# SomeBottle/LinearProgramming

Hardware: AMD Instinct MI355X
Metric: Simplex pivots/sec + HBM GB/s fraction, dense m=16384×n=32768 fp64, 1/2/4/8 GPU (higher is better)
Workload: dtype f64

## Files before the change

### linearprogramming_amd/csrc/lpg_ctx.hip

```cpp
#include <hip/hip_runtime.h>
#include <rccl/rccl.h>

#include <dlfcn.h>
#include <unistd.h>
#include <math.h>
#include <stdarg.h>
#include <stdio.h>
#include <stdlib.h>
#include <string.h>

#include <algorithm>
#include <vector>

#include "../../include/lpg.h"
#include "lpg_internal.h"

using namespace lpg;

namespace {

thread_local char g_err[512];

struct TimingRing {
    std::vector<hipEvent_t> ev;
// ... 238 lines not shown
    t.used = 0;
    return 0;
}

static int timing_mark(lpg_ctx *c, int which, int updated = 1) {
    TimingRing &t = c->tr;
    if (which == 0 && t.used * 3 + 3 > (int)t.ev.size()) {
        int rc = timing_flush(c);
        if (rc) return rc;
    }
    HIPCHK(c, hipEventRecord(t.ev[3 * t.used + which], c->stream));
    if (which == 2) t.upd[t.used++] = (char)updated;
    return 0;
}


static Defer defer_of(const lpg_ctx *c, int q) {
    Defer d;
    d.Pbuf = c->Pbuf;
    d.Cbuf = c->Cbuf;
    d.cs = c->cs;
    d.rq = c->rq;
    d.rqg = c->rqg;
    d.basis = c->basis;
    d.logk = c->logk;
    d.logr = c->logr;
    d.zrow = c->zrow;
    d.kq = c->kq;
    d.lv = c->lv;
    d.colmap = c->colmap;
    d.inv = c->inv;
    d.mul = c->mul;
    d.pv = c->pv;
    d.q = q;
    d.on = c->defer_k > 0 ? 1 : 0;
    return d;
}

static bool reorders(const lpg_ctx *c) { return c->defer_k > 0 && c->fast_pivot && c->colmap && !c->no_reorder; }

#ifdef LPG_TEST_HOOKS
static int inject_pending_fault(lpg_ctx *c) {
    switch (c->inject_what) {
        case 1: HIPCHK(c, hipMemsetAsync(&c->st->npend, 0x7f, sizeof(int64_t), c->stream)); break;
        case 2: HIPCHK(c, hipMemsetAsync(c->kq, 0xff, sizeof(int64_t), c->stream)); break;
        case 3: HIPCHK(c, hipMemsetAsync(c->lv, 0xff, sizeof(int64_t), c->stream)); break;
        case 4: HIPCHK(c, hipMemsetAsync(c->rq, 0x7f, sizeof(int64_t), c->stream)); break;
        case 5: {
            HIPCHK(c, hipStreamSynchronize(c->stream));
            int64_t np = 0;
            HIPCHK(c, hipMemcpy(&np, &c->st->npend, sizeof np, hipMemcpyDeviceToHost));
            np += 1;
            HIPCHK(c, hipMemcpy(&c->st->npend, &np, sizeof np, hipMemcpyHostToDevice));
            break;
        }
        default: break;
    }
    return 0;
}

#endif

static int flush_launch(lpg_ctx *c) {
    int rc;
    const bool re = reorders(c);
#ifdef LPG_TEST_HOOKS
    if (c->inject_flush >= 0 && c->nflush == c->inject_flush && (rc = inject_pending_fault(c))) return rc;
#endif
    c->nflush++;
    const int unit = (c->block_region && c->reg_valid && c->move_unit) ? 1 : 0;
    if (launch_swap_plan(lau(c), geo(c), c->st, defer_of(c, 0), c->colmap, c->inv, c->pairs, re ? 1 : 0, c->defer_k) ||
        (re && launch_move_cols(lau(c), geo(c), c->st, defer_of(c, 0), c->pairs, unit)))
        return fail(c, LPG_ERR_DEVICE, "swap plan launch failed");
#ifdef LPG_TEST_HOOKS
    if (c->inject_rbad >= 0 && c->nflush == c->inject_rbad + 1)
        HIPCHK(c, hipMemsetAsync(&c->st->rbad, 0x01, sizeof(uint32_t), c->stream));
#endif
    if (c->timing && ((rc = timing_mark(c, 0)) || (rc = timing_mark(c, 1)))) return rc;
    const int32_t *tl = (c->block_region && c->reg_valid && re && c->tlive_on && c->skip) ? c->tlive : nullptr;
    c->block_region = false;
    if (launch_flush_main(lau(c), geo(c), c->st, defer_of(c, 0), c->pend, c->skip, c->flush_variant, c->flush_xcd, tl))
        return fail(c, LPG_ERR_DEVICE, "flush launch failed");
    if (c->timing && (rc = timing_mark(c, 2, 2))) return rc;
    if (launch_flush_tail(lau(c), geo(c), c->st, defer_of(c, 0), c->pend, !re))
        return fail(c, LPG_ERR_DEVICE, "flush launch failed");
    if (re) {
        const Defer D = defer_of(c, 0);
        if (launch_fill_cols(lau(c), geo(c), c->pairs, c->st, &D, flush_kmax_supported(c->defer_k),
                             c->reg ? c->bcol0 : nullptr))
            return fail(c, LPG_ERR_DEVICE, "fill launch failed");
        c->permuted = true;
    }
    c->pend = 0;
    return 0;
}

static int materialize(lpg_ctx *c) {
    if (c->defer_k == 0 || c->pend == 0) return 0;
    return flush_launch(c);
}

static int canonicalize(lpg_ctx *c) {
    int rc = materialize(c);
    c->reg_valid = false;
    if (rc || !c->permuted) return rc;
    const int64_t rows = c->nloc + c->nobj;
    if (!c->tmp) {
        c->tmp_rows = std::min<int64_t>(rows, 512);
        HIPCHK(c, hipMalloc(&c->tmp, (size_t)c->tmp_rows * c->ld * sizeof(double)));
    }
    const Geo g = geo(c);
    for (int64_t i0 = 0; i0 < rows; i0 += c->tmp_rows) {
        const int64_t nr = std::min(c->tmp_rows, rows - i0);
        if (launch_gather_rows(lau(c), g, c->inv, c->tmp, i0, nr)) return fail(c, LPG_ERR_DEVICE, "gather launch failed");
        HIPCHK(c, hipMemcpy2DAsync(c->T + i0 * c->ld, c->ld * sizeof(double), c->tmp, c->ld * sizeof(double),
                                   c->ncols * sizeof(double), nr, hipMemcpyDeviceToDevice, c->stream));
    }
    if (launch_iota(lau(c), c->colmap, c->ld) || launch_iota(lau(c), c->inv, c->ld))
        return fail(c, LPG_ERR_DEVICE, "iota launch failed");
    c->permuted = false;
    return 0;
}


static int cand_per_rank(const lpg_ctx *c) { return (c->defer_k > 0 && c->fast_pivot) ? c->nsel_d : c->nsel; }

static int64_t prow_count(const lpg_ctx *c) { return (c->ncols + 1) & ~(int64_t)1; }

static int exchange_candidates(lpg_ctx *c) {
    if (!has_comm(c)) return 0;
    return comm_allgather(c, c->part, c->cand, sizeof(Cand) * (size_t)cand_per_rank(c));
}

static int clear_candidates(lpg_ctx *c) {
    if (c->nsel_d > c->nsel)
        HIPCHK(c, hipMemsetAsync(c->part + c->nsel, 0xff, (size_t)(c->nsel_d - c->nsel) * sizeof(Cand), c->stream));
    return 0;
}

static int region_setup(lpg_ctx *c);

static int bootstrap(lpg_ctx *c, int rule) {
    int rc = canonicalize(c);
    if (rc || (rc = region_setup(c)) || (rc = clear_candidates(c))) return rc;
    HIPCHK(c, hipMemsetAsync(c->st->slot, 0, sizeof(c->st->slot), c->stream));
    const Geo g = geo(c);
    if (launch_price(lau(c), g, rule, 0, c->st, 0, c->P, c->C[0], c->pp, c->pc, c->npp))
        return fail(c, LPG_ERR_DEVICE, "price launch failed");
    if (launch_select(lau(c), g, rule, true, c->st, 0, 0, c->P, c->C[1], c->C[0], c->pp, c->npp, c->basis,
                      c->part, c->nsel, 0, -1, c->pc, c->skip, defer_of(c, 0)))
        return fail(c, LPG_ERR_DEVICE, "select launch failed");
    if ((rc = exchange_candidates(c))) return rc;
    c->par = 0;
    c->booted = true;
    c->boot_rule = rule;
    c->x_from_cand = true;
    return 0;
}

static int bootstrap_forced(lpg_ctx *c, int rule, int64_t k, int64_t r) {
    int rc = canonicalize(c);
    if (rc || (rc = region_setup(c)) || (rc = clear_candidates(c))) return rc;
    HIPCHK(c, hipMemsetAsync(c->st->slot, 0, sizeof(c->st->slot), c->stream));
    if (launch_select(lau(c), geo(c), rule, true, c->st, 0, 0, c->P, c->C[1], c->C[0], c->pp, c->npp, c->basis,
                      c->part, c->nsel, k, r, c->pc, c->skip, defer_of(c, 0)))
        return fail(c, LPG_ERR_DEVICE, "select launch failed");
    if ((rc = exchange_candidates(c))) return rc;
    c->par = 0;
    c->booted = true;
    c->boot_rule = rule;
    c->x_from_cand = true;
    return 0;
}

static constexpr int kGraphPivots = 32;
// ... 1427 lines not shown
```

### linearprogramming_amd/csrc/lpg_internal.h

```cpp
#pragma once
#include <stddef.h>
#include <stdint.h>

namespace lpg {

constexpr int kBlock = 256;
constexpr int kMaxSelBlocks = 512;
#ifndef LPG_DEFER_MAX
#define LPG_DEFER_MAX 128
#endif

enum : int32_t { RUNNING = 0, OPTIMAL = 1, UNBOUNDED = 2, INFEASIBLE = 3, ITER_LIMIT = 4, NUMERIC = 5 };
enum : int { RULE_DANTZIG = 0, RULE_BLAND = 1 };

struct Slot {
    int64_t k;
    int64_t r;
    int32_t status;
    int32_t pad0;
    int64_t dpend;
};

struct DevState {
    Slot    slot[2];
// ... 48 lines not shown

struct Cand {
    double  theta;
    double  piv;
    int64_t key;
    int64_t row;
};

struct PricePart {
    double  v;
    int64_t j;
    int32_t cls;
    int32_t pad;
};

struct Geo {
    double *T;
    int64_t ld;
    int64_t nloc;
    int64_t nobj;
    int64_t ncols;
    int64_t nact;
    int64_t row0;
    int64_t m;
    double  eps_piv, eps_opt;
};

struct Launch {
    void   *stream;
};

int launch_generate(const Launch &L, const Geo &g, int64_t n, uint64_t seed, int kind, int64_t *basis_dev);
int launch_objective_chain(const Launch &L, const Geo &g, const double *cb, const double *acc_in, double *acc_out);
int launch_objective_finish(const Launch &L, const Geo &g, const double *acc, const double *cost, int64_t orow);
int launch_price(const Launch &L, const Geo &g, int rule, int mode, const DevState *st, int s,
                 const double *P, const double *Cs, PricePart *pp, int *pc, int npp, bool defer = false,
                 const int32_t *colmap = nullptr, const int32_t *inv = nullptr);
int launch_prep(const Launch &L, const Geo &g, int rule, bool fuse_price, DevState *st, int s,
                const Cand *cand, int ncand, double *P, const double *Cs, PricePart *pp, int *pc, int npp,
                const Defer &D);
int launch_select(const Launch &L, const Geo &g, int rule, bool first, DevState *st, int s, int s1,
                  const double *P, const double *Cs, double *Cs1, const PricePart *pp, int npp,
                  const int64_t *basis, Cand *part, int nsel, int64_t force_k, int64_t force_r,
                  const int *pc, int skip, const Defer &D);
constexpr int kPivotThreads = 256;
int pivot_d_blocks(const Geo &g, int which, int nt);
int launch_pivot_d(const Launch &L, const Geo &g, int rule, DevState *st, int s, int s1, Cand *part, int nsel,
                   double *P, const double *Cs, double *Cs1, PricePart *pp, int npp, const int64_t *basis,
                   const Defer &D, int nt);
int launch_prep_dm(const Launch &L, const Geo &g, int rule, DevState *st, int s, const Cand *cand, int ncand,
                   double *P, const double *Cs, int npp_d, const Defer &D);
int launch_prep_x(const Launch &L, const Geo &g, int rule, DevState *st, int s, const Cand *cand, int ncand,
                  double *P, const double *Cs, PricePart *pp, int npp_d, const Defer &D, const Xch &X);
int launch_select_x(const Launch &L, const Geo &g, int rule, DevState *st, int s, int s1, const double *Cs,
                    double *Cs1, const PricePart *pp, int npp, const int64_t *basis, Cand *part, int nsel,
                    const Defer &D, const Xch &X);
int64_t xch_bytes(int64_t ld, int world, int nblk, int nx, int64_t *offF, int64_t *offC, int64_t *offG);
int launch_select_dm(const Launch &L, const Geo &g, int rule, DevState *st, int s, int s1, const double *Cs,
                     double *Cs1, const PricePart *pp, int npp, const int64_t *basis, Cand *part, int nsel,
                     const Defer &D);
int block_records_bytes(int nwg);
int block_geometry(const Geo &g, int ks, int cus, int want, int *nwg, int *cw, int *rw, size_t *lds);
struct RegionGeo {
    int nwg, cw, rw, nsp, cwx;
    size_t lds;
};
struct RegionArgs {
    const int32_t *live;
    int64_t nlive;
    const int64_t *bcol0;
    int nsp, cwx;
};
int block_geometry_region(const Geo &g, int ks, int cus, int want, int64_t nlive, RegionGeo *out);
int launch_region_build(const Launch &L, const Geo &g, DevState *st, const int64_t *basis, const int32_t *inv,
                        int32_t *mark, int32_t *live, int64_t *bcol0, int64_t nlive, int32_t *tlive);
int launch_region_check(const Launch &L, const Geo &g, const int64_t *basis, const int32_t *inv, int *ok);
int launch_pivot_block(const Launch &L, const Geo &g, int rule, DevState *st, int s0, int q0, int n, Cand *part,
                       int ncand, const Cand *cin, int ncin, const double *Cs0, double *Cs1, const Defer &D,
                       void *rec, uint32_t tag0, int nwg, int cw, int rw, int ks, size_t lds, uint32_t cl,
                       const Xch *X = nullptr, uint32_t xtag0 = 0, const RegionArgs *R = nullptr);
int launch_flush(const Launch &L, const Geo &g, DevState *st, const Defer &D, int kmax, int skip, int which);
int launch_flush_main(const Launch &L, const Geo &g, DevState *st, const Defer &D, int kmax, int skip, int which,
                      int xcd = -1, const int32_t *tlive = nullptr);
int launch_flush_tail(const Launch &L, const Geo &g, DevState *st, const Defer &D, int kmax, bool reset = true);
__host__ __device__ inline int64_t flush_tail_rows(int64_t rows, int64_t nloc) {
    return (rows > 0 && nloc >= 8 * rows && rows >= 64) ? rows / 4 : 0;
}
__host__ __device__ inline int64_t flush_nitems(int64_t ntiles, int64_t rows, int64_t nloc) {
    const int64_t tr = flush_tail_rows(rows, nloc);
    if (rows < 0) rows = -rows;
    if (!tr) return ntiles * ((nloc + rows - 1) / rows);
    const int64_t t0 = ((nloc + rows - 1) / rows - 2) * rows;
    return ntiles * (t0 / rows) + ntiles * ((nloc - t0 + tr - 1) / tr);
}
__host__ __device__ inline void flush_item(int64_t item, int64_t ntiles, int64_t rows, int64_t nloc, int64_t &tile,
                                           int64_t &i0, int64_t &i1) {
    const int64_t tr = flush_tail_rows(rows, nloc);
    if (rows < 0) rows = -rows;
    const int64_t t0 = tr ? ((nloc + rows - 1) / rows - 2) * rows : nloc;
    const int64_t nbig = ntiles * (t0 / rows);
    tile = item % ntiles;
    if (!tr || item < nbig) {
        i0 = (item / ntiles) * rows;
        i1 = i0 + rows;
    } else {
        i0 = t0 + ((item - nbig) / ntiles) * tr;
        i1 = i0 + tr;
    }
    if (i1 > nloc) i1 = nloc;
}
struct FlushX {
    int64_t ntiles, nloc;
    int32_t H;
    int32_t rb;
    int32_t rs;
    int32_t tt;
    int32_t on;
    int32_t tq;
};
struct FlushXGroup {
    int64_t r0, r1, ntg, nsb, ttg, nq, qrows, count;
};
__host__ __device__ inline FlushXGroup flushx_group(const FlushX &f, int g) {
    FlushXGroup o{};
    const int b = g / f.H, h = g % f.H;
    o.r0 = (int64_t)b * f.rb;
    o.r1 = o.r0 + f.rb < f.nloc ? o.r0 + f.rb : f.nloc;
    o.ntg = h < f.ntiles ? (f.ntiles - h + f.H - 1) / f.H : 0;
    if (o.r0 >= f.nloc || o.ntg == 0) return o;
    o.nsb = (o.r1 - o.r0 + f.rs - 1) / f.rs;
    const int64_t ls = (o.r1 - o.r0) - (o.nsb - 1) * f.rs;
    const int64_t tq = f.tq > 0 ? f.tq : 4;
    o.qrows = ((ls + tq - 1) / tq + 15) / 16 * 16;
    o.nq = (ls + o.qrows - 1) / o.qrows;
    o.ttg = f.tt < o.ntg ? f.tt : o.ntg;
    o.count = (o.nsb - 1) * o.ntg + (o.ntg - o.ttg) + o.nq * o.ttg;
    return o;
}
__host__ __device__ inline void flushx_item(const FlushX &f, const FlushXGroup &G, int g, int64_t it, int64_t &tile,
                                            int64_t &i0, int64_t &i1) {
    const int h = g % f.H;
    int64_t j;
    const int64_t full = (G.nsb - 1) * G.ntg;
    const int64_t base = G.r0 + (G.nsb - 1) * f.rs;
    if (it < full) {
        j = G.ntg - 1 - it % G.ntg;
        i0 = G.r0 + (it / G.ntg) * f.rs;
        i1 = i0 + f.rs;
    } else if (it - full < G.ntg - G.ttg) {
        j = G.ntg - 1 - (it - full);
        i0 = base;
        i1 = G.r1;
    } else {
        const int64_t k = it - full - (G.ntg - G.ttg);
        j = G.ttg - 1 - k / G.nq;
        i0 = base + (k % G.nq) * G.qrows;
        i1 = i0 + G.qrows;
    }
    if (i1 > G.r1) i1 = G.r1;
    tile = h + (int64_t)f.H * j;
}
int flush_kmax_supported(int k);
int launch_swap_plan(const Launch &L, const Geo &g, DevState *st, const Defer &D, int32_t *colmap, int32_t *inv,
                     int32_t *pairs, int plan, int kmax);
constexpr int kPairW = 4;
int launch_move_cols(const Launch &L, const Geo &g, const DevState *st, const Defer &D, const int32_t *pairs,
                     int unit);
int launch_fill_cols(const Launch &L, const Geo &g, const int32_t *pairs, DevState *st = nullptr,
                     const Defer *D = nullptr, int kmax = 0, int64_t *bcol0 = nullptr);
int launch_gather_rows(const Launch &L, const Geo &g, const int32_t *inv, double *tmp, int64_t i0, int64_t nr);
int launch_iota(const Launch &L, int32_t *a, int64_t n);
int launch_update(const Launch &L, const Geo &g, DevState *st, int s, const double *P, const double *Cs,
                  int64_t *basis, int64_t *logk, int64_t *logr, int variant, int skip);

int launch_dual_rows(const Launch &L, const Geo &g, Cand *part, int nsel);
int launch_dual_row_d(const Launch &L, const Geo &g, DevState *st, int s, const Cand *rc, int nrc, Cand *cp,
                      double *R, const double *Pprev, const double *Cprev, const Defer &D, bool mr);
int launch_dual_ratio(const Launch &L, const Geo &g, const DevState *st, int s, const double *R, Cand *cp);
int launch_dual_col_d(const Launch &L, const Geo &g, DevState *st, int s, const Cand *cp, const double *R, double *Cs,
                      Cand *rc, int nrc_out, const Defer &D);
int launch_dual_pivot(const Launch &L, const Geo &g, DevState *st, int s, Cand *part, int nsel, PricePart *pp,
                      int *pc, int npp, int skip, double *P, double *Cs, bool price_only = false);

#ifdef LPG_PHASES
int debug_phases(unsigned long long *out, int reset);
int debug_block_phases(unsigned long long *out);
#endif
int price_blocks(const Geo &g);
int update_variants();
int update_auto_variant(const Geo &g);

}
```

### linearprogramming_amd/csrc/lpg_kernels.hip

```cpp
#include <hip/hip_runtime.h>
#include <math.h>

#include <stddef.h>
#include <stdlib.h>

#include <algorithm>

#include "lpg_internal.h"
#include "lpg_device.h"

namespace lpg {



static inline uint64_t splitmix64_host(uint64_t x) {
    uint64_t z = x + 0x9E3779B97F4A7C15ull;
    z = (z ^ (z >> 30)) * 0xBF58476D1CE4E5B9ull;
    z = (z ^ (z >> 27)) * 0x94D049BB133111EBull;
    return z ^ (z >> 31);
}
static inline uint64_t subkey(uint64_t seed, uint64_t which) {
    return splitmix64_host(seed ^ (which * 0xD1B54A32D192ED03ull));
}

// ... 1652 lines not shown
#pragma unroll
            for (int w = 0; w < WPB; w++) sum += wsum[w];
            touched += (unsigned long long)sum * (unsigned long long)(i1 - i0);
        }
        const int nb = (int)((i1 - i0 + 15) / 16);
        auto cload = [&](d2 (&cr)[PER], int s) {
#pragma unroll
            for (int u = 0; u < PER; u++) {
                const int e = threadIdx.x + u * NTH;
                const int q = e >> 3, rr = 2 * (e & 7);
                const int64_t row = i0 + 16 * s + rr;
                d2 v = d2{0.0, 0.0};
                if (s < nb && q < np && row < i1 && (NPC % NTH == 0 || e < NPC))
                    v = *(const d2 *)(Cbuf + (int64_t)q * cs + row);
                cr[u] = -v;
            }
        };
        auto cstore = [&](const d2 (&cr)[PER], int s) {
#pragma unroll
            for (int u = 0; u < PER; u++)
                if (NPC % NTH == 0 || threadIdx.x + u * NTH < NPC) *(d2 *)(&sC[s % NB][2 * (threadIdx.x + u * NTH)]) = cr[u];
        };
        for (int s = 0; s < NB - 1; s++) {
            d2 cr[PER];
            cload(cr, s);
            cstore(cr, s);
        }
        d2 cn[PER];
        cload(cn, NB - 1);
        auto tload = [&](d2 (&x)[4], int s) {
#pragma unroll
            for (int r = 0; r < 4; r++) {
                const int64_t row = i0 + 16 * s + lk + 4 * r;
                x[r] = (ok && row < i1) ? __builtin_nontemporal_load((const d2 *)(T + row * ld + cl)) : d2{0.0, 0.0};
            }
        };
        d2 t[4];
        tload(t, 0);
        for (int s = 0; s < nb; s++) {
            d2 tn[4];
            if (s + 1 < nb) tload(tn, s + 1);
            __syncthreads();
            cstore(cn, s + NB - 1);
            cload(cn, s + NB);
            if (wlive) {
                d4 ae = d4{t[0].x, t[1].x, t[2].x, t[3].x};
                d4 ao = d4{t[0].y, t[1].y, t[2].y, t[3].y};
                const double *sa = &sC[s % NB][lk * 16 + lc];
                double a0 = sa[0], a1 = sa[64];
#pragma unroll
                for (int gq = 0; gq < G; gq += 2) {
                    double n0 = 0.0, n1 = 0.0;
                    if (gq + 2 < G) {
                        n0 = sa[(gq + 2) * 64];
                        n1 = sa[(gq + 3) * 64];
                    }
                    __builtin_amdgcn_sched_barrier(0);
                    ae = __builtin_amdgcn_mfma_f64_16x16x4f64(a0, be[gq], ae, 0, 0, 0);
                    ao = __builtin_amdgcn_mfma_f64_16x16x4f64(a0, bo[gq], ao, 0, 0, 0);
                    ae = __builtin_amdgcn_mfma_f64_16x16x4f64(a1, be[gq + 1], ae, 0, 0, 0);
                    ao = __builtin_amdgcn_mfma_f64_16x16x4f64(a1, bo[gq + 1], ao, 0, 0, 0);
                    __builtin_amdgcn_sched_barrier(0);
                    a0 = n0;
                    a1 = n1;
                }
#pragma unroll
                for (int r = 0; r < 4; r++) {
                    const int64_t row = i0 + 16 * s + lk + 4 * r;
                    if (ok && row < i1) __builtin_nontemporal_store(d2{ae[r], ao[r]}, (d2 *)(T + row * ld + cl));
                }
            }
#pragma unroll
            for (int r = 0; r < 4; r++) t[r] = tn[r];
        }
    }
    if (threadIdx.x == 0 && touched) atomicAdd(&st->touched, touched);
}

template <int K>
__global__ __launch_bounds__(kBlock) void k_flush_pivot_rows(double *__restrict__ T, Geo g,
                                                             const DevState *__restrict__ st,
                                                             const double *__restrict__ Pbuf,
                                                             const double *__restrict__ mul,
                                                             const int64_t *__restrict__ rq) {
    static_assert((K == 64 || K == 96 || K == 128) && K <= LPG_DEFER_MAX && kBlock == 256,
                  "4 waves x K/16 groups of 4 rows");
    constexpr bool LM = K == 64;
    constexpr int PW = K / (kBlock / 64);
    constexpr int MT = LM ? K * K / kBlock : 1;
    __shared__ double sP[K][64];
    __shared__ __attribute__((aligned(32))) double sM[LM ? K * K : 4];
    __shared__ __attribute__((aligned(32))) double sMg[LM ? 1 : kBlock / 64][LM ? 1 : K][4];
    const int np = (int)st->npend;
    if (np <= 0) return;
    const int c = threadIdx.x & 63, w = threadIdx.x >> 6;
    const int64_t j = (int64_t)blockIdx.x * 64 + c;
    const bool ok = j < g.ncols;
    {
        double v[PW], m[MT];
#pragma unroll
        for (int k = 0; k < PW; k++) {
            const int u = w + 4 * k;
            v[k] = (ok && u < np) ? Pbuf[(int64_t)u * g.ld + j] : 0.0;
        }
#pragma unroll
        for (int k = 0; k < MT; k++) {
            const int e = threadIdx.x + kBlock * k;
            m[k] = (LM && e / K < np) ? mul[(e / K) * LPG_DEFER_MAX + e % K] : 0.0;
        }
#pragma unroll
        for (int k = 0; k < PW; k++) sP[w + 4 * k][c] = v[k];
        if (LM) {
#pragma unroll
            for (int k = 0; k < MT; k++) sM[threadIdx.x + kBlock * k] = m[k];
        }
    }
    const int64_t ru = c < np ? rq[c] : -1;
    const int64_t ru1 = K > 64 && 64 + c < np ? rq[64 + c] : -1;
    __syncthreads();
#pragma unroll 1
    for (int k = 0; k < K / 16; k++) {
        const int grp = (k & 1) ? 8 * (k >> 1) + 7 - w : 8 * (k >> 1) + w;
        const int q0 = 4 * grp;
        if (q0 >= np) continue;
        double x0 = sP[q0][c], x1 = sP[q0 + 1][c], x2 = sP[q0 + 2][c], x3 = sP[q0 + 3][c];
        if (!LM) {
#pragma unroll
            for (int k = 0; k < (LM ? 1 : (K + 63) / 64); k++) {
                const int u = c + 64 * k;
                if (u < K) {
                    const d4 m = *(const d4 *)(mul + (u < np ? u : 0) * LPG_DEFER_MAX + q0);
                    *(d4 *)&sMg[LM ? 0 : w][LM ? 0 : u][0] = u < np ? m : d4{0.0, 0.0, 0.0, 0.0};
                }
            }
        }
        auto m4 = [&](int u) {
            return LM ? *(const d4 *)(sM + u * K + q0) : *(const d4 *)&sMg[LM ? 0 : w][LM ? 0 : u][0];
        };
        if (q0 + 1 < np) {
            const double p = sP[q0 + 1][c];
            const d4 m = m4(q0 + 1);
            x0 = fma(m[0], p, x0);
        }
        if (q0 + 2 < np) {
            const double p = sP[q0 + 2][c];
            const d4 m = m4(q0 + 2);
            x0 = fma(m[0], p, x0);
            x1 = fma(m[1], p, x1);
        }
        if (q0 + 3 < np) {
            const double p = sP[q0 + 3][c];
            const d4 m = m4(q0 + 3);
            x0 = fma(m[0], p, x0);
            x1 = fma(m[1], p, x1);
            x2 = fma(m[2], p, x2);
        }
#pragma unroll 2
        for (int u = q0 + 4; u < np; u++) {
            const double p = sP[u][c];
            const d4 m = m4(u);
            x0 = fma(m[0], p, x0);
            x1 = fma(m[1], p, x1);
            x2 = fma(m[2], p, x2);
            x3 = fma(m[3], p, x3);
        }
        const double xs[4] = {x0, x1, x2, x3};
#pragma unroll
        for (int i = 0; i < 4; i++) {
            const int q = q0 + i;
            if (q >= np) break;
            const int64_t r = q < 64 ? (int64_t)rdl64((uint64_t)ru, q) : (int64_t)rdl64((uint64_t)ru1, q - 64);
            if (r < 0) continue;
            if (__ballot(c > q && ru == r)) continue;
            if (K > 64 && __ballot(64 + c > q && ru1 == r)) continue;
            if (ok) T[r * g.ld + j] = xs[i];
        }
    }
}


constexpr int kMulBlocks = 8;
constexpr int kPlanNT = LPG_DEFER_MAX;
__global__ __launch_bounds__(kPlanNT) void k_swap_plan(DevState *__restrict__ st, const int64_t *__restrict__ kq,
                                                  const int64_t *__restrict__ lv, const int64_t *__restrict__ rq,
                                                  const double *__restrict__ Cbuf, int64_t cs,
                                                  int32_t *__restrict__ colmap, int32_t *__restrict__ inv,
                                                  int32_t *__restrict__ pairs, double *__restrict__ mul, int plan,
                                                  const double *__restrict__ pv, int64_t nloc, int64_t ncols, int kmax) {
    const int64_t np64 = st->npend;
    const bool npbad = np64 < 0 || np64 > kmax;
    const int np = npbad ? 0 : (int)np64;
    {
        const int q = threadIdx.x;
        int what = npbad ? 1 : 0;
        int64_t val = np64;
        if (!npbad && q < np) {
            const int64_t x = plan ? kq[q] : 1, y = plan ? lv[q] : 1, r = rq[q];
            if (x < 1 || x >= ncols) what = 2, val = x;
            else if (y < 1 || y >= ncols) what = 3, val = y;
            else if (r < -1 || r >= nloc) what = 4, val = r;
        }
        __shared__ int first;
        if (q == 0) first = kPlanNT;
        __syncthreads();
        if (what) atomicMin(&first, q);
        if (__syncthreads_or(what != 0)) {
            if (blockIdx.x == 0 && q == first) {
                if (st->stall == 0) {
                    st->stall_info[0] = what;
                    st->stall_info[1] = q;
                    st->stall_info[2] = val;
                    st->stall_info[3] = np64;
                    st->stall = kStallPending;
                }
                st->npend = 0;
                if (pairs) pairs[0] = 0;
                for (int u = 0; u < 2; u++)
                    if (st->slot[u].status == RUNNING) st->slot[u].status = NUMERIC;
            }
            return;
        }
    }
    if (blockIdx.x > 0) {
        constexpr int UB = LPG_DEFER_MAX / kMulBlocks;
        const int q = threadIdx.x;
        const int u0 = (blockIdx.x - 1) * UB;
        const int64_t r = q < np ? rq[q] : -1;
        double v[UB];
#pragma unroll
        for (int k = 0; k < UB; k++) {
            const int u = u0 + k;
            const bool on = u > q && u < np && r >= 0;
            const double c = Cbuf[(int64_t)(on ? u : 0) * cs + (on ? r : 0)];
            v[k] = on ? -c : 0.0;
        }
#pragma unroll
        for (int k = 0; k < UB; k++)
            if (u0 + k < np) mul[(u0 + k) * LPG_DEFER_MAX + q] = v[k];
        return;
    }
    if (!plan) return;
    const int q = threadIdx.x;
    const int64_t x = q < np ? kq[q] : -1, y = q < np ? lv[q] : -1, rx = q < np ? rq[q] : -1;
    const bool pos = q >= np || pv[q] > 0.0;
    __shared__ int64_t sx[kPlanNT], sy[kPlanNT];
    sx[q] = x;
    sy[q] = y;
    bool inE = q < np, inL = q < np;
    int fx = q, fy = q;
    bool fxe = true, fye = false;
    const bool allpos = __syncthreads_count(!pos) == 0;
    if (q == 0 && np > 0 && !allpos) st->rbad = 1;
#pragma unroll 8
    for (int u = 0; u < np; u++) {
        const int64_t a = sx[u], b = sy[u];
        if (u > q) {
            if (a == x || b == x) inE = false;
            if (a == y || b == y) inL = false;
        } else if (u < q) {
            if (a == x && u < fx) { fx = u; fxe = true; }
            if (b == x && u < fx) { fx = u; fxe = false; }
            if (a == y && u < fy) { fy = u; fye = true; }
            if (b == y && u < fy) { fy = u; fye = false; }
        }
    }
    inE = inE && fxe && allpos;
    inL = inL && !fye && allpos;
    constexpr int NW = kPlanNT / 64;
    const int lane = q & 63, wv = q >> 6;
    const unsigned long long me = __ballot(inE), ml = __ballot(inL);
    __shared__ int cE[NW], cL[NW];
    if (lane == 0) {
        cE[wv] = __popcll(me);
        cL[wv] = __popcll(ml);
    }
    __syncthreads();
    int oE = 0, oL = 0, n = 0;
#pragma unroll
    for (int w = 0; w < NW; w++) {
        oE += w < wv ? cE[w] : 0;
        oL += w < wv ? cL[w] : 0;
        n += cE[w];
    }
    const unsigned long long below = (lane == 0) ? 0ull : (~0ull >> (64 - lane));
    const int ie = oE + __popcll(me & below), il = oL + __popcll(ml & below);
    __shared__ int64_t eE[kPlanNT], eL[kPlanNT], eR[kPlanNT], eRL[kPlanNT];
    if (inE) {
        eE[ie] = x;
        eR[ie] = rx;
    }
    if (inL) {
        eL[il] = y;
        eRL[il] = rx;
    }
    __syncthreads();
    if (q < n) {
        const int64_t ce = eE[q], cl = eL[q];
        const int32_t a = inv[ce], b = inv[cl];
        pairs[1 + kPairW * q] = a;
        pairs[2 + kPairW * q] = b;
        pairs[3 + kPairW * q] = (int32_t)eR[q];
        pairs[4 + kPairW * q] = (int32_t)eRL[q];
        colmap[a] = (int32_t)cl;
        colmap[b] = (int32_t)ce;
        inv[cl] = a;
        inv[ce] = b;
    }
    if (q == 0) pairs[0] = n;
}

__global__ __launch_bounds__(kBlock) void k_move_cols(double *__restrict__ T, Geo g, const DevState *__restrict__ st,
                                                      double *__restrict__ Pbuf, const int32_t *__restrict__ pairs,
                                                      int npb, int unit) {
    const int n = pairs[0];
    if (n == 0) return;
    const int nrb = (int)gridDim.x - npb;
    if ((int)blockIdx.x >= nrb) {
        const int np = (int)st->npend;
        const int nt = npb * (int)gridDim.y * kBlock;
        for (int e = (((int)blockIdx.x - nrb) * (int)gridDim.y + (int)blockIdx.y) * kBlock + threadIdx.x; e < np * n;
             e += nt) {
            const int q = e / n, p = e - q * n;
            double *Pq = Pbuf + (int64_t)q * g.ld;
            const int32_t a = pairs[1 + kPairW * p], b = pairs[2 + kPairW * p];
            Pq[a] = Pq[b];
            Pq[b] = 0.0;
        }
        return;
    }
    const int64_t i = (int64_t)blockIdx.x * kBlock + threadIdx.x;
    if (i >= g.nloc + g.nobj) return;
    const bool obj = i >= g.nloc;
    double *row = T + i * g.ld;
    for (int p0 = 16 * blockIdx.y; p0 < n; p0 += 16 * gridDim.y) {
        double va[16], vb[16];
        int ia[16], ib[16], rl[16];
#pragma unroll
        for (int u = 0; u < 16; u++) {
            ia[u] = p0 + u < n ? pairs[1 + kPairW * (p0 + u)] : 0;
            ib[u] = p0 + u < n ? pairs[2 + kPairW * (p0 + u)] : 0;
            rl[u] = p0 + u < n ? pairs[4 + kPairW * (p0 + u)] : -1;
        }
#pragma unroll
        for (int u = 0; u < 16; u++) {
            vb[u] = (unit && !obj) ? ((int64_t)rl[u] == i ? 1.0 : 0.0) : row[ib[u]];
            va[u] = obj ? row[ia[u]] : 0.0;
        }
#pragma unroll
        for (int u = 0; u < 16; u++)
            if (p0 + u < n) {
                row[ia[u]] = vb[u];
                if (obj) row[ib[u]] = va[u];
            }
    }
}

__device__ __forceinline__ void end_block(DevState *st, const Defer &D, int kmax, bool spare_zero = false,
                                          int64_t ld = 0) {
    const int q = threadIdx.x;
    if (spare_zero) {
        const int64_t L = q < kmax ? D.lv[q] : 0;
        if (L > 0) {
            double *col = D.Pbuf + D.inv[L];
            for (int u = 0; u < kmax; u++) col[(int64_t)u * ld] = 0.0;
        }
        __syncthreads();
    }
    if (q == 0) {
        st->npend = 0;
        st->fwork = 0;
    }
    if (q < 8) st->gwork[q] = 0;
    for (int u = q; u < kmax; u += blockDim.x) {
        D.rq[u] = kNoSlot;
        if (D.kq) D.kq[u] = 0;
        if (D.lv) D.lv[u] = 0;
    }
}

__global__ __launch_bounds__(kBlock) void k_end_block(DevState *__restrict__ st, Defer D, int kmax) {
    end_block(st, D, kmax);
}

__global__ __launch_bounds__(kBlock) void k_fill_cols(double *__restrict__ T, Geo g, const int32_t *__restrict__ pairs,
                                                      DevState *__restrict__ st, Defer D, int kmax,
                                                      int64_t *__restrict__ bcol0) {
    if (st && blockIdx.x == 0 && blockIdx.y == 0) end_block(st, D, kmax, bcol0 != nullptr, g.ld);
    if (bcol0 && blockIdx.y == 0) {
        for (int64_t r = (int64_t)blockIdx.x * kBlock + threadIdx.x; r < g.m; r += (int64_t)gridDim.x * kBlock) {
            const int64_t v = D.basis[r];
            bcol0[r] = (v << 32) | (int64_t)(uint32_t)D.inv[v];
        }
    }
    const int n = pairs[0];
    const int64_t i = (int64_t)blockIdx.x * kBlock + threadIdx.x;
    if (i >= g.nloc || n == 0) return;
    double *row = T + i * g.ld;
    for (int p = blockIdx.y; p < n; p += gridDim.y)
        row[pairs[2 + kPairW * p]] = (i == (int64_t)pairs[3 + kPairW * p]) ? 1.0 : 0.0;
}

int launch_swap_plan(const Launch &L, const Geo &g, DevState *st, const Defer &D, int32_t *colmap, int32_t *inv,
                     int32_t *pairs, int plan, int kmax) {
    kmax = flush_kmax_supported(kmax);
    if (!kmax || (plan && !pairs)) return -1;
    hipLaunchKernelGGL(k_swap_plan, dim3(1 + kMulBlocks), dim3(kPlanNT), 0, (hipStream_t)L.stream, st, D.kq, D.lv, D.rq,
                       D.Cbuf, D.cs, colmap, inv, pairs, D.mul, plan, D.pv, g.nloc, g.ncols, kmax);
    return hipGetLastError() == hipSuccess ? 0 : -1;
}

int launch_move_cols(const Launch &L, const Geo &g, const DevState *st, const Defer &D, const int32_t *pairs,
                     int unit) {
    const int64_t rows = g.nloc + g.nobj;
    const int npb = (LPG_DEFER_MAX * LPG_DEFER_MAX + 4 * kBlock - 1) / (4 * kBlock);
    hipLaunchKernelGGL(k_move_cols, dim3((unsigned)((rows + kBlock - 1) / kBlock + npb), 4), dim3(kBlock), 0,
                       (hipStream_t)L.stream, g.T, g, st, D.Pbuf, pairs, npb, unit);
    return hipGetLastError() == hipSuccess ? 0 : -1;
}

int launch_fill_cols(const Launch &L, const Geo &g, const int32_t *pairs, DevState *st, const Defer *D, int kmax,
                     int64_t *bcol0) {
    if (st && (!D || !D->rq || kmax < 1 || kmax > LPG_DEFER_MAX)) return -1;
    if (bcol0 && (!st || !D->basis || !D->inv || !D->lv || !D->Pbuf)) return -1;
    hipLaunchKernelGGL(k_fill_cols, dim3((unsigned)std::max<int64_t>((g.nloc + kBlock - 1) / kBlock, 1), 4), dim3(kBlock),
                       0, (hipStream_t)L.stream, g.T, g, pairs, st, D ? *D : Defer{}, kmax, bcol0);
    return hipGetLastError() == hipSuccess ? 0 : -1;
}

__global__ __launch_bounds__(kBlock) void k_gather_rows(const double *__restrict__ T, Geo g,
                                                        const int32_t *__restrict__ inv, double *__restrict__ tmp,
                                                        int64_t i0, int64_t nr) {
    const int64_t r = blockIdx.y;
    if (r >= nr) return;
    const double *src = T + (i0 + r) * g.ld;
    double *dst = tmp + r * g.ld;
    for (int64_t j = (int64_t)blockIdx.x * kBlock + threadIdx.x; j < g.ncols; j += (int64_t)gridDim.x * kBlock)
        dst[j] = src[inv[j]];
}

int launch_gather_rows(const Launch &L, const Geo &g, const int32_t *inv, double *tmp, int64_t i0, int64_t nr) {
    const int64_t tiles = std::min<int64_t>((g.ncols + kBlock - 1) / kBlock, 64);
    hipLaunchKernelGGL(k_gather_rows, dim3((unsigned)tiles, (unsigned)nr), dim3(kBlock), 0, (hipStream_t)L.stream,
                       g.T, g, inv, tmp, i0, nr);
    return hipGetLastError() == hipSuccess ? 0 : -1;
}

__global__ void k_iota(int32_t *a, int64_t n) {
    for (int64_t j = (int64_t)blockIdx.x * blockDim.x + threadIdx.x; j < n; j += (int64_t)gridDim.x * blockDim.x)
        a[j] = (int32_t)j;
}

int launch_iota(const Launch &L, int32_t *a, int64_t n) {
    hipLaunchKernelGGL(k_iota, dim3(256), dim3(kBlock), 0, (hipStream_t)L.stream, a, n);
    return hipGetLastError() == hipSuccess ? 0 : -1;
}

int flush_kmax_supported(int k) {
    if (k <= 8) return 8;
    if (k <= 16) return 16;
    if (k <= 32) return 32;
    if (k <= 64) return 64;
    if (k <= 96) return 96;
    if (k <= 128 && k <= LPG_DEFER_MAX) return 128;
    return 0;
}

static_assert(offsetof(DevState, fwork) == offsetof(DevState, npend) + sizeof(int64_t),
              "launch_flush clears npend and fwork with one memset");

int launch_flush_tail(const Launch &L, const Geo &g, DevState *st, const Defer &D, int kmax, bool reset) {
    kmax = flush_kmax_supported(kmax);
    if (!kmax) return -1;
    hipStream_t stream = (hipStream_t)L.stream;
    const int64_t ntiles_p = (g.ncols + 63) / 64;
#ifdef LPG_PIVROWS96
    if (kmax == 96)
        hipLaunchKernelGGL(k_flush_pivot_rows<96>, dim3((unsigned)ntiles_p), dim3(kBlock), 0, stream, g.T, g, st,
                           D.Pbuf, D.mul, D.rq);
    else
#endif
    if (kmax > 64)
        hipLaunchKernelGGL(k_flush_pivot_rows<128>, dim3((unsigned)ntiles_p), dim3(kBlock), 0, stream, g.T, g, st,
                           D.Pbuf, D.mul, D.rq);
    else
        hipLaunchKernelGGL(k_flush_pivot_rows<64>, dim3((unsigned)ntiles_p), dim3(kBlock), 0, stream, g.T, g, st,
                           D.Pbuf, D.mul, D.rq);
    if (hipGetLastError() != hipSuccess) return -1;
    if (!reset) return 0;
    hipLaunchKernelGGL(k_end_block, dim3(1), dim3(kBlock), 0, stream, st, D, kmax);
    return hipGetLastError() == hipSuccess ? 0 : -1;
}

int launch_flush(const Launch &L, const Geo &g, DevState *st, const Defer &D, int kmax, int skip, int variant) {
    int rc = launch_swap_plan(L, g, st, D, nullptr, nullptr, nullptr, 0, kmax);
    if (!rc) rc = launch_flush_main(L, g, st, D, kmax, skip, variant);
    return rc ? rc : launch_flush_tail(L, g, st, D, kmax);
}

static bool flush_tail_on() {
    static const int on = [] {
        const char *v = getenv("LPG_FLUSH_TAIL");
        return v ? atoi(v) != 0 : 1;
    }();
    return on != 0;
}

static int64_t flush_rows_env(int64_t def) {
    static const int64_t v = [] {
        const char *e = getenv("LPG_FLUSH_ROWS");
        const long r = e ? atol(e) : 0;
        return (int64_t)((r >= 64 && r <= 8192 && r % 64 == 0) ? r : 0);
    }();
    return v ? v : def;
}

static int64_t flush_minitems_env(int64_t def) {
    static const int64_t v = [] {
        const char *e = getenv("LPG_FLUSH_MINITEMS");
        const long r = e ? atol(e) : 0;
        return (int64_t)((r >= 256 && r <= 65536) ? r : 0);
    }();
    return v ? v : def;
}

static int64_t env_range(const char *name, int64_t lo, int64_t hi) {
    const char *e = getenv(name);
    const long long v = e ? atoll(e) : 0;
    return (v >= lo && v <= hi) ? (int64_t)v : 0;
}

static FlushX flushx_plan(int64_t ntiles, int64_t nloc, int kmax, int64_t nblocks, int xcd) {
    FlushX X{};
    if (xcd == 0 || nloc < 1 || ntiles < 1 || (xcd < 0 && (nloc < 1024 || ntiles < 64))) return X;
    static const int64_t cb = env_range("LPG_FLUSH_CB", 256, 65536) * 1024;
    static const int64_t ttf = env_range("LPG_FLUSH_XTAIL", 1, 1 << 20);
    static const int64_t tqf = env_range("LPG_FLUSH_XPIECES", 1, 64);
    const int64_t budget = cb ? cb : (int64_t)2048 * 1024;
    auto band = [&](int H) { return ((nloc + 8 / H - 1) / (8 / H) + 15) / 16 * 16; };
    int H = 1;
    if (xcd == 11 || xcd == 12 || xcd == 14 || xcd == 18)
        H = xcd - 10;
    else
        for (int h : {8, 4, 2})
            if (band(h) * kmax * 8 <= budget) {
                H = h;
                break;
            }
    X.ntiles = ntiles;
    X.nloc = nloc;
    X.H = H;
    const int64_t rb = band(H);
    const int64_t nsb = std::max<int64_t>(1, (rb * kmax * 8 + budget - 1) / budget);
    X.rb = (int32_t)rb;
    X.rs = (int32_t)std::min<int64_t>(rb, ((rb + nsb - 1) / nsb + 15) / 16 * 16);
    X.tt = (int32_t)(ttf ? ttf : std::max<int64_t>(1, nblocks / 8 / 2));
    X.tq = (int32_t)(tqf ? tqf : 8);
    X.on = 1;
    return X;
}

int launch_flush_main(const Launch &L, const Geo &g, DevState *st, const Defer &D, int kmax, int skip, int which,
                      int xcd, const int32_t *tlive) {
    kmax = flush_kmax_supported(kmax);
    if (!kmax) return -1;
    if (which < 0) which = 1;
    hipStream_t stream = (hipStream_t)L.stream;
    if (kmax >= 64) which = 1;
    if (which == 1) {
        constexpr int kW64 = 8;
        static const int w96 = env_range("LPG_FLUSH_W96", 4, 4) == 4 ? 4 : 8;
        const bool wide = kmax == 64 || (kmax == 96 && w96 == 8);
        const int tw = wide ? 32 * kW64 : 128;
        const int64_t ntiles = (g.ncols + tw - 1) / tw;
// ... 58 lines not shown
```

Baseline: 29660.

## Fold unit-column fill into move_cols and pivot-row flush, drop fill_cols kernel

```diff
diff --git a/linearprogramming_amd/csrc/lpg_ctx.hip b/linearprogramming_amd/csrc/lpg_ctx.hip
--- a/linearprogramming_amd/csrc/lpg_ctx.hip
+++ b/linearprogramming_amd/csrc/lpg_ctx.hip
@@ -344,15 +344,12 @@
     if (launch_flush_main(lau(c), geo(c), c->st, defer_of(c, 0), c->pend, c->skip, c->flush_variant, c->flush_xcd, tl))
         return fail(c, LPG_ERR_DEVICE, "flush launch failed");
     if (c->timing && (rc = timing_mark(c, 2, 2))) return rc;
-    if (launch_flush_tail(lau(c), geo(c), c->st, defer_of(c, 0), c->pend, !re))
+    if (launch_flush_tail(lau(c), geo(c), c->st, defer_of(c, 0), c->pend, false, re ? c->pairs : nullptr))
         return fail(c, LPG_ERR_DEVICE, "flush launch failed");
-    if (re) {
-        const Defer D = defer_of(c, 0);
-        if (launch_fill_cols(lau(c), geo(c), c->pairs, c->st, &D, flush_kmax_supported(c->defer_k),
-                             c->reg ? c->bcol0 : nullptr))
-            return fail(c, LPG_ERR_DEVICE, "fill launch failed");
-        c->permuted = true;
-    }
+    if (launch_end_block(lau(c), geo(c), c->st, defer_of(c, 0), flush_kmax_supported(c->defer_k),
+                         (re && c->reg) ? c->bcol0 : nullptr))
+        return fail(c, LPG_ERR_DEVICE, "end-of-block launch failed");
+    if (re) c->permuted = true;
     c->pend = 0;
     return 0;
 }
diff --git a/linearprogramming_amd/csrc/lpg_internal.h b/linearprogramming_amd/csrc/lpg_internal.h
--- a/linearprogramming_amd/csrc/lpg_internal.h
+++ b/linearprogramming_amd/csrc/lpg_internal.h
@@ -154,7 +154,8 @@
 int launch_flush(const Launch &L, const Geo &g, DevState *st, const Defer &D, int kmax, int skip, int which);
 int launch_flush_main(const Launch &L, const Geo &g, DevState *st, const Defer &D, int kmax, int skip, int which,
                       int xcd = -1, const int32_t *tlive = nullptr);
-int launch_flush_tail(const Launch &L, const Geo &g, DevState *st, const Defer &D, int kmax, bool reset = true);
+int launch_flush_tail(const Launch &L, const Geo &g, DevState *st, const Defer &D, int kmax, bool reset = true,
+                      const int32_t *pairs = nullptr);
 __host__ __device__ inline int64_t flush_tail_rows(int64_t rows, int64_t nloc) {
     return (rows > 0 && nloc >= 8 * rows && rows >= 64) ? rows / 4 : 0;
 }
@@ -238,8 +239,7 @@
 constexpr int kPairW = 4;
 int launch_move_cols(const Launch &L, const Geo &g, const DevState *st, const Defer &D, const int32_t *pairs,
                      int unit);
-int launch_fill_cols(const Launch &L, const Geo &g, const int32_t *pairs, DevState *st = nullptr,
-                     const Defer *D = nullptr, int kmax = 0, int64_t *bcol0 = nullptr);
+int launch_end_block(const Launch &L, const Geo &g, DevState *st, const Defer &D, int kmax, int64_t *bcol0 = nullptr);
 int launch_gather_rows(const Launch &L, const Geo &g, const int32_t *inv, double *tmp, int64_t i0, int64_t nr);
 int launch_iota(const Launch &L, int32_t *a, int64_t n);
 int launch_update(const Launch &L, const Geo &g, DevState *st, int s, const double *P, const double *Cs,
diff --git a/linearprogramming_amd/csrc/lpg_kernels.hip b/linearprogramming_amd/csrc/lpg_kernels.hip
--- a/linearprogramming_amd/csrc/lpg_kernels.hip
+++ b/linearprogramming_amd/csrc/lpg_kernels.hip
@@ -1758,7 +1758,8 @@
                                                              const DevState *__restrict__ st,
                                                              const double *__restrict__ Pbuf,
                                                              const double *__restrict__ mul,
-                                                             const int64_t *__restrict__ rq) {
+                                                             const int64_t *__restrict__ rq,
+                                                             const int32_t *__restrict__ pairs) {
     static_assert((K == 64 || K == 96 || K == 128) && K <= LPG_DEFER_MAX && kBlock == 256,
                   "4 waves x K/16 groups of 4 rows");
     constexpr bool LM = K == 64;
@@ -1767,11 +1768,13 @@
     __shared__ double sP[K][64];
     __shared__ __attribute__((aligned(32))) double sM[LM ? K * K : 4];
     __shared__ __attribute__((aligned(32))) double sMg[LM ? 1 : kBlock / 64][LM ? 1 : K][4];
+    constexpr int kNotIb = -2;
     const int np = (int)st->npend;
     if (np <= 0) return;
     const int c = threadIdx.x & 63, w = threadIdx.x >> 6;
     const int64_t j = (int64_t)blockIdx.x * 64 + c;
     const bool ok = j < g.ncols;
+    int eb = kNotIb;
     {
         double v[PW], m[MT];
 #pragma unroll
@@ -1783,6 +1786,19 @@
         for (int k = 0; k < MT; k++) {
             const int e = threadIdx.x + kBlock * k;
             m[k] = (LM && e / K < np) ? mul[(e / K) * LPG_DEFER_MAX + e % K] : 0.0;
+        }
+        if (pairs) {
+            int *sE = (int *)&sP[0][0];
+            if (w == 0) sE[c] = kNotIb;
+            __syncthreads();
+            const int n = pairs[0];
+            for (int p = threadIdx.x; p < n; p += kBlock) {
+                const int32_t b = pairs[2 + kPairW * p];
+                if ((b >> 6) == (int)blockIdx.x) sE[b & 63] = pairs[3 + kPairW * p];
+            }
+            __syncthreads();
+            eb = sE[c];
+            __syncthreads();
         }
 #pragma unroll
         for (int k = 0; k < PW; k++) sP[w + 4 * k][c] = v[k];
@@ -1849,7 +1865,7 @@
             if (r < 0) continue;
             if (__ballot(c > q && ru == r)) continue;
             if (K > 64 && __ballot(64 + c > q && ru1 == r)) continue;
-            if (ok) T[r * g.ld + j] = xs[i];
+            if (ok) T[r * g.ld + j] = eb == kNotIb ? xs[i] : ((int64_t)eb == r ? 1.0 : 0.0);
         }
     }
 }
@@ -2010,11 +2026,12 @@
     double *row = T + i * g.ld;
     for (int p0 = 16 * blockIdx.y; p0 < n; p0 += 16 * gridDim.y) {
         double va[16], vb[16];
-        int ia[16], ib[16], rl[16];
+        int ia[16], ib[16], re[16], rl[16];
 #pragma unroll
         for (int u = 0; u < 16; u++) {
             ia[u] = p0 + u < n ? pairs[1 + kPairW * (p0 + u)] : 0;
             ib[u] = p0 + u < n ? pairs[2 + kPairW * (p0 + u)] : 0;
+            re[u] = p0 + u < n ? pairs[3 + kPairW * (p0 + u)] : -1;
             rl[u] = p0 + u < n ? pairs[4 + kPairW * (p0 + u)] : -1;
         }
 #pragma unroll
@@ -2027,6 +2044,7 @@
             if (p0 + u < n) {
                 row[ia[u]] = vb[u];
                 if (obj) row[ib[u]] = va[u];
+                else if (!unit) row[ib[u]] = (int64_t)re[u] == i ? 1.0 : 0.0;
             }
     }
 }
@@ -2054,26 +2072,15 @@
     }
 }
 
-__global__ __launch_bounds__(kBlock) void k_end_block(DevState *__restrict__ st, Defer D, int kmax) {
-    end_block(st, D, kmax);
-}
-
-__global__ __launch_bounds__(kBlock) void k_fill_cols(double *__restrict__ T, Geo g, const int32_t *__restrict__ pairs,
-                                                      DevState *__restrict__ st, Defer D, int kmax,
-                                                      int64_t *__restrict__ bcol0) {
-    if (st && blockIdx.x == 0 && blockIdx.y == 0) end_block(st, D, kmax, bcol0 != nullptr, g.ld);
-    if (bcol0 && blockIdx.y == 0) {
-        for (int64_t r = (int64_t)blockIdx.x * kBlock + threadIdx.x; r < g.m; r += (int64_t)gridDim.x * kBlock) {
+__global__ __launch_bounds__(kBlock) void k_end_block(DevState *__restrict__ st, Defer D, int kmax,
+                                                      int64_t *__restrict__ bcol0, int64_t ld, int64_t m) {
+    if (blockIdx.x == 0) end_block(st, D, kmax, bcol0 != nullptr, ld);
+    if (bcol0) {
+        for (int64_t r = (int64_t)blockIdx.x * kBlock + threadIdx.x; r < m; r += (int64_t)gridDim.x * kBlock) {
             const int64_t v = D.basis[r];
             bcol0[r] = (v << 32) | (int64_t)(uint32_t)D.inv[v];
         }
     }
-    const int n = pairs[0];
-    const int64_t i = (int64_t)blockIdx.x * kBlock + threadIdx.x;
-    if (i >= g.nloc || n == 0) return;
-    double *row = T + i * g.ld;
-    for (int p = blockIdx.y; p < n; p += gridDim.y)
-        row[pairs[2 + kPairW * p]] = (i == (int64_t)pairs[3 + kPairW * p]) ? 1.0 : 0.0;
 }
 
 int launch_swap_plan(const Launch &L, const Geo &g, DevState *st, const Defer &D, int32_t *colmap, int32_t *inv,
@@ -2094,12 +2101,12 @@
     return hipGetLastError() == hipSuccess ? 0 : -1;
 }
 
-int launch_fill_cols(const Launch &L, const Geo &g, const int32_t *pairs, DevState *st, const Defer *D, int kmax,
-                     int64_t *bcol0) {
-    if (st && (!D || !D->rq || kmax < 1 || kmax > LPG_DEFER_MAX)) return -1;
-    if (bcol0 && (!st || !D->basis || !D->inv || !D->lv || !D->Pbuf)) return -1;
-    hipLaunchKernelGGL(k_fill_cols, dim3((unsigned)std::max<int64_t>((g.nloc + kBlock - 1) / kBlock, 1), 4), dim3(kBlock),
-                       0, (hipStream_t)L.stream, g.T, g, pairs, st, D ? *D : Defer{}, kmax, bcol0);
+int launch_end_block(const Launch &L, const Geo &g, DevState *st, const Defer &D, int kmax, int64_t *bcol0) {
+    if (!st || !D.rq || kmax < 1 || kmax > LPG_DEFER_MAX) return -1;
+    if (bcol0 && (!D.basis || !D.inv || !D.lv || !D.Pbuf)) return -1;
+    const int64_t nb = bcol0 ? std::min<int64_t>(std::max<int64_t>((g.m + kBlock - 1) / kBlock, 1), 64) : 1;
+    hipLaunchKernelGGL(k_end_block, dim3((unsigned)nb), dim3(kBlock), 0, (hipStream_t)L.stream, st, D, kmax, bcol0, g.ld,
+                       g.m);
     return hipGetLastError() == hipSuccess ? 0 : -1;
 }
 
@@ -2144,7 +2151,8 @@
 static_assert(offsetof(DevState, fwork) == offsetof(DevState, npend) + sizeof(int64_t),
               "launch_flush clears npend and fwork with one memset");
 
-int launch_flush_tail(const Launch &L, const Geo &g, DevState *st, const Defer &D, int kmax, bool reset) {
+int launch_flush_tail(const Launch &L, const Geo &g, DevState *st, const Defer &D, int kmax, bool reset,
+                      const int32_t *pairs) {
     kmax = flush_kmax_supported(kmax);
     if (!kmax) return -1;
     hipStream_t stream = (hipStream_t)L.stream;
@@ -2152,19 +2160,18 @@
 #ifdef LPG_PIVROWS96
     if (kmax == 96)
         hipLaunchKernelGGL(k_flush_pivot_rows<96>, dim3((unsigned)ntiles_p), dim3(kBlock), 0, stream, g.T, g, st,
-                           D.Pbuf, D.mul, D.rq);
+                           D.Pbuf, D.mul, D.rq, pairs);
     else
 #endif
     if (kmax > 64)
         hipLaunchKernelGGL(k_flush_pivot_rows<128>, dim3((unsigned)ntiles_p), dim3(kBlock), 0, stream, g.T, g, st,
-                           D.Pbuf, D.mul, D.rq);
+                           D.Pbuf, D.mul, D.rq, pairs);
     else
         hipLaunchKernelGGL(k_flush_pivot_rows<64>, dim3((unsigned)ntiles_p), dim3(kBlock), 0, stream, g.T, g, st,
-                           D.Pbuf, D.mul, D.rq);
+                           D.Pbuf, D.mul, D.rq, pairs);
     if (hipGetLastError() != hipSuccess) return -1;
     if (!reset) return 0;
-    hipLaunchKernelGGL(k_end_block, dim3(1), dim3(kBlock), 0, stream, st, D, kmax);
-    return hipGetLastError() == hipSuccess ? 0 : -1;
+    return launch_end_block(L, g, st, D, kmax, nullptr);
 }
 
 int launch_flush(const Launch &L, const Geo &g, DevState *st, const Defer &D, int kmax, int skip, int variant) {
```

Result: faster. 30020, median of 6 (+1.2%).
